# xxlong0/ESTDepth

Hardware: AMD Instinct MI355X
Metric: depth frames/sec (seq_len=5, 480x640, D=64) (higher is better)
Workload: dtype f32

## Files before the change

### estdepth_amd/csrc/conv2d_wino2.hip

```cpp
#include <hip/hip_runtime.h>
#include <stdint.h>
#include <stdlib.h>
#include <type_traits>

#include "estd_hip.h"
#include "estd_common.h"

#ifndef ESTD_C2W2ABL
#define ESTD_C2W2ABL 0
#endif

namespace {

typedef float f32x4 __attribute__((ext_vector_type(4)));
typedef float f32x2 __attribute__((ext_vector_type(2)));
typedef unsigned int u32x4 __attribute__((__vector_size__(16)));
constexpr unsigned OOB_OFFSET = 0xFFFFFF00u;

constexpr int TH = 8, TW = 16;
constexpr int TROWS = 16;
constexpr int NSTEP = 8;
#ifndef ESTD_C2W2_PFS
#define ESTD_C2W2_PFS 8
#endif
#ifndef ESTD_C2W2_WD
#define ESTD_C2W2_WD 2
#endif
#ifndef ESTD_C2W2_INLOOP
#define ESTD_C2W2_INLOOP 1
#endif
#ifndef ESTD_C2W2_INLOOP_PFS
#define ESTD_C2W2_INLOOP_PFS 4
#endif
#ifndef ESTD_C2W2_INLOOP_W0
#define ESTD_C2W2_INLOOP_W0 4
#endif
#ifndef ESTD_C2W2_SCHED
#define ESTD_C2W2_SCHED 2
#endif
constexpr int WD = ESTD_C2W2_WD, WR = 4;

__device__ __forceinline__ float4 as_float4(u32x4 v) { float4 f; __builtin_memcpy(&f, &v, 16); return f; }
__device__ __forceinline__ u32x4 as_u32x4(float4 f) { u32x4 v; __builtin_memcpy(&v, &f, 16); return v; }
__device__ __forceinline__ float4 f4_sub(float4 a, float4 b) { return make_float4(a.x - b.x, a.y - b.y, a.z - b.z, a.w - b.w); }
__device__ __forceinline__ float4 f4_add(float4 a, float4 b) { return make_float4(a.x + b.x, a.y + b.y, a.z + b.z, a.w + b.w); }
__device__ __forceinline__ __amdgpu_buffer_rsrc_t make_rsrc(const float* base, size_t elems)
{
    return __builtin_amdgcn_make_buffer_rsrc(const_cast<float*>(base), 0, (int)(elems * 4), 0x00020000);
}
__device__ __forceinline__ void lds_barrier() { asm volatile("s_waitcnt lgkmcnt(0)\n\ts_barrier" ::: "memory"); }

template <int DIL>
__global__ __launch_bounds__(256, 2) void conv2d_wino2_kernel(const estd_conv2d_desc p, int tiles_w, int tiles_h, int total_items)
{
    constexpr int IN_H = TH + 2 * DIL, IN_W = TW + 2 * DIL;
    constexpr bool INLOOP = ESTD_C2W2_INLOOP != 0 && (DIL == 1 || ESTD_C2W2_INLOOP == 2);
    constexpr int PITCH = DIL == 1 ? IN_W + 1 : IN_W;
    constexpr int SLOT_BYTES = TROWS * PITCH * 128;
    constexpr int SH_BYTES = 4 * PITCH * 128;
    constexpr int LOADERS = IN_W * 8;
    auto lds_off = [](int row, int col, int chunk) { return (row * PITCH + col) * 128 + ((chunk ^ ((col >> 1) & 7)) << 4); };
    extern __shared__ __attribute__((aligned(16))) char smem[];

    const int tid = threadIdx.x;
    const int lane = tid & 63;
    const int wave = __builtin_amdgcn_readfirstlane(tid >> 6);
    const int rpp = wave >> 1, nt = wave & 1;
    const int g = lane >> 4, i = lane & 15;
    const int blk_rp = (i >= 4 && i < 12) ? 1 : 0;
    const int cb = i < 4 ? i : i < 12 ? i - 4 : i - 8;
    const int rp = 2 * rpp + blk_rp;
    const int row_a = DIL == 1 ? 2 * rp : (rp & 1) + 4 * (rp >> 1);
    const int col_b = DIL == 1 ? 2 * cb : (cb & 1) + 4 * (cb >> 1);
    const int H = p.H, W = p.W, Cin = p.cin, Cout = p.cout;
    const int nchunks = Cin >> 5;
    const int tiles_per_group = p.N * tiles_h * tiles_w;
    const int wlane = lane * 16 + nt * 1024;

    int u, u_end;
    {
        const int G = gridDim.x, bid = blockIdx.x;
        const int r = ((G & 7) == 0) ? (bid & 7) * (G >> 3) + (bid >> 3) : bid;
        u = (int)((long long)total_items * r / G);
        u_end = (int)((long long)total_items * (r + 1) / G);
    }
    if (u >= u_end) return;

    const size_t img_in = (size_t)H * W * Cin, img_out = (size_t)H * W * Cout;
    const bool loader = tid < LOADERS;
    const int lzx = tid >> 3, lc = tid & 7;
    const int wbase = loader ? lds_off(0, lzx, lc) : 0;

    int aoff[4];
#pragma unroll
    for (int q = 0; q < 4; ++q) aoff[q] = lds_off(rp, col_b + DIL * q, g);

    auto decode = [&](int item, int& grp, int& n, int& th0, int& tw0) {
        grp = item / tiles_per_group;
        int t = item - grp * tiles_per_group;
        const int twi = t % tiles_w; t /= tiles_w;
        const int thi = t % tiles_h; n = t / tiles_h;
        th0 = thi * TH; tw0 = twi * TW;
    };
    auto brick_offsets = [&](int th0, int tw0, unsigned (&voff)[IN_H], bool enable) {
        const int gx = tw0 - DIL + lzx;
        const bool colok = enable && loader && (unsigned)gx < (unsigned)W;
        const unsigned base = (unsigned)(gx * Cin + lc * 4) * 4u;
        const unsigned rowbytes = (unsigned)(W * Cin) * 4u;
#pragma unroll
        for (int zy = 0; zy < IN_H; ++zy) {
            const int gy = th0 - DIL + zy;
            const bool rowok = (unsigned)gy < (unsigned)H;
            voff[zy] = (colok && rowok) ? base + (unsigned)gy * rowbytes : OOB_OFFSET;
        }
    };

    int grp, n, th0, tw0;
    decode(u, grp, n, th0, tw0);
    unsigned voff[IN_H];
    brick_offsets(th0, tw0, voff, true);
    __amdgpu_buffer_rsrc_t rs_in = make_rsrc(p.in + (size_t)n * img_in, img_in);
    float4 pf[IN_H];
#pragma unroll
    for (int zy = 0; zy < IN_H; ++zy) pf[zy] = as_float4(__builtin_amdgcn_raw_buffer_load_b128(rs_in, voff[zy], 0, 0));

    const size_t wgrp_elems = (size_t)nchunks * NSTEP * 4 * 2 * 256;
    float4 bq[WR][4];
    {
        const __amdgpu_buffer_rsrc_t rs_w0 = make_rsrc(p.w_wino + (size_t)grp * wgrp_elems, wgrp_elems);
#pragma unroll
        for (int s = 0; s < WD; ++s)
#pragma unroll
            for (int sw = 0; sw < 4; ++sw) bq[s][sw] = as_float4(__builtin_amdgcn_raw_buffer_load_b128(rs_w0, wlane, (s * 4 + sw) * 2048, 0));
    }
    const float floor_b = p.relu_before_residual ? 0.f : ESTD_NO_FLOOR;
    const float floor_a = p.relu_after_residual ? 0.f : ESTD_NO_FLOOR;

    int k = 0;
    if (INLOOP) {
        if (loader && !(ESTD_C2W2ABL & 2)) {
#pragma unroll
            for (int w = 0; w < 4; ++w) {
                const int a = DIL == 1 ? 2 * w : (w & 1) + 4 * (w >> 1);
                const float4 d0 = pf[a], d1 = pf[a + DIL], d2 = pf[a + 2 * DIL], d3 = pf[a + 3 * DIL];
                *reinterpret_cast<float4*>(smem + wbase + (0 * 4 + w) * PITCH * 128) = f4_sub(d0, d2);
                *reinterpret_cast<float4*>(smem + wbase + (1 * 4 + w) * PITCH * 128) = f4_add(d1, d2);
                *reinterpret_cast<float4*>(smem + wbase + (2 * 4 + w) * PITCH * 128) = f4_sub(d2, d1);
                *reinterpret_cast<float4*>(smem + wbase + (3 * 4 + w) * PITCH * 128) = f4_sub(d1, d3);
            }
        }
    }
    while (true) {
        const __amdgpu_buffer_rsrc_t rs_w = make_rsrc(p.w_wino + (size_t)grp * wgrp_elems, wgrp_elems);
        const int cbase = grp * 32 + nt * 16 + 4 * g;
        const float4 sc4 = *reinterpret_cast<const float4*>(p.scale + cbase), sh4 = *reinterpret_cast<const float4*>(p.shift + cbase);
        f32x4 acc[4][4];

        const bool has_next_item = (u + 1 < u_end);
        int ngrp = grp, nn_ = n, nth0 = th0, ntw0 = tw0;
        if (has_next_item) decode(u + 1, ngrp, nn_, nth0, ntw0);
        const __amdgpu_buffer_rsrc_t rs_wni = make_rsrc(p.w_wino + (size_t)ngrp * wgrp_elems, wgrp_elems);

        auto write_rows = [&](char* slot, int w0, int w1) {
            if (loader && !(ESTD_C2W2ABL & 2)) {
#pragma unroll
                for (int w = 0; w < 4; ++w) {
                    if (w < w0 || w >= w1) continue;
                    const int a = DIL == 1 ? 2 * w : (w & 1) + 4 * (w >> 1);
                    const float4 d0 = pf[a], d1 = pf[a + DIL], d2 = pf[a + 2 * DIL], d3 = pf[a + 3 * DIL];
                    *reinterpret_cast<float4*>(slot + wbase + (0 * 4 + w) * PITCH * 128) = f4_sub(d0, d2);
                    *reinterpret_cast<float4*>(slot + wbase + (1 * 4 + w) * PITCH * 128) = f4_add(d1, d2);
                    *reinterpret_cast<float4*>(slot + wbase + (2 * 4 + w) * PITCH * 128) = f4_sub(d2, d1);
                    *reinterpret_cast<float4*>(slot + wbase + (3 * 4 + w) * PITCH * 128) = f4_sub(d1, d3);
                }
            }
        };
        auto write_row_sh = [&](char* slot, int w, int sh_) {
            if (loader && !(ESTD_C2W2ABL & 2)) {
                const int a = DIL == 1 ? 2 * w : (w & 1) + 4 * (w >> 1);
                const float4 d0 = pf[a], d1 = pf[a + DIL], d2 = pf[a + 2 * DIL], d3 = pf[a + 3 * DIL];
                const float4 v = sh_ == 0 ? f4_sub(d0, d2) : sh_ == 1 ? f4_add(d1, d2) : sh_ == 2 ? f4_sub(d2, d1) : f4_sub(d1, d3);
                *reinterpret_cast<float4*>(slot + wbase + (sh_ * 4 + w) * PITCH * 128) = v;
            }
        };
        auto chunk_body = [&](auto first_c, const int c) {
            constexpr bool FIRST = decltype(first_c)::value;
            const int sb = (k & 1) * SLOT_BYTES;
            char* slot = smem + sb;
            if (!INLOOP) write_rows(slot, 0, 4);
            lds_barrier();

            const bool last_chunk = (c + 1 == nchunks);
            int pf_soff = (c + 1) * 128;
            if (last_chunk) {
                brick_offsets(nth0, ntw0, voff, has_next_item);
                if (nn_ != n) rs_in = make_rsrc(p.in + (size_t)nn_ * img_in, img_in);
                pf_soff = 0;
            }
            const int wbase_q = c * NSTEP * 4;
            const __amdgpu_buffer_rsrc_t rs_wx = last_chunk ? rs_wni : rs_w;
            const int wnext_q = last_chunk ? 0 : wbase_q + NSTEP * 4;

            int ao[4];
#pragma unroll
            for (int q = 0; q < 4; ++q) ao[q] = aoff[q] + sb;
            auto load_rows = [&](int st, float4 (&Rr)[4]) {
#pragma unroll
                for (int q = 0; q < 4; ++q)
                    Rr[q] = *reinterpret_cast<const float4*>(smem + ((st & 1) ? (ao[q] ^ 64) : ao[q]) + (st >> 1) * SH_BYTES);
            };
            auto xform2 = [&](const float4 (&Rr)[4], int h, f32x2 (&o)[4]) {
                f32x2 r[4];
#pragma unroll
                for (int q = 0; q < 4; ++q) r[q] = h == 0 ? (f32x2){Rr[q].x, Rr[q].y} : (f32x2){Rr[q].z, Rr[q].w};
                if (ESTD_C2W2ABL & 128) { o[0] = r[0]; o[1] = r[1]; o[2] = r[2]; o[3] = r[3]; }
                else { o[0] = r[0] - r[2]; o[1] = r[1] + r[2]; o[2] = r[2] - r[1]; o[3] = r[1] - r[3]; }
            };
            f32x2 T[2][4];
            float4 R[4];
            load_rows(0, R);
            xform2(R, 0, T[0]);
            xform2(R, 1, T[1]);
            load_rows(1, R);
            __builtin_amdgcn_sched_barrier(0);

#pragma clang loop unroll(full)
            for (int st = 0; st < NSTEP; ++st) {
                const int sh = st >> 1;
                f32x2 Tn[2][4];
                if (ESTD_C2W2_SCHED == 2) {
                    constexpr int PFS = INLOOP ? ESTD_C2W2_INLOOP_PFS : ESTD_C2W2_PFS;
                    const int r0 = PFS != 8 ? (st < PFS ? st * IN_H / PFS : IN_H) : DIL == 1 ? (st == 0 ? 0 : st + 1) : (3 * st + 1) / 2;
                    const int r1 = PFS != 8 ? (st < PFS ? (st + 1) * IN_H / PFS : IN_H)
                                            : DIL == 1 ? ((st == 0 || st == NSTEP - 1) ? r0 + 2 : r0 + 1) : (3 * (st + 1) + 1) / 2;
                    const bool wr = INLOOP && st >= ESTD_C2W2_INLOOP_W0 && (!last_chunk || has_next_item);
                    constexpr int WN = NSTEP - ESTD_C2W2_INLOOP_W0;
                    static_assert(!INLOOP || WN == 4, "quarter schedule: one row pair of the next chunk per step");
#pragma unroll
                    for (int h = 0; h < 2; ++h) {
#pragma unroll
                        for (int e = 0; e < 2; ++e) {
                            const int qk = 2 * h + e;
                            if (!(ESTD_C2W2ABL & 8)) {
                                const int tgt = st + WD;
                                bq[tgt % WR][qk] = tgt < NSTEP
                                    ? as_float4(__builtin_amdgcn_raw_buffer_load_b128(rs_w, wlane, (wbase_q + tgt * 4 + qk) * 2048, 0))
                                    : as_float4(__builtin_amdgcn_raw_buffer_load_b128(rs_wx, wlane, (wnext_q + (tgt - NSTEP) * 4 + qk) * 2048, 0));
                            }
#pragma unroll
                            for (int r = r0 + (r1 - r0) * qk / 4; r < r0 + (r1 - r0) * (qk + 1) / 4; ++r)
                                pf[r] = as_float4(__builtin_amdgcn_raw_buffer_load_b128(rs_in, voff[r], pf_soff, 0));
                            if (wr) write_row_sh(smem + (((k + 1) & 1) * SLOT_BYTES), st - ESTD_C2W2_INLOOP_W0, qk);
                            __builtin_amdgcn_sched_barrier(0);
#pragma unroll
                            for (int sw = 0; sw < 4; ++sw) {
                                const float4 b4 = bq[(ESTD_C2W2ABL & 8) ? 0 : st % WR][sw];
                                const float b = h == 0 ? (e == 0 ? b4.x : b4.y) : (e == 0 ? b4.z : b4.w);
                                const bool first_product = FIRST && (st & 1) == 0 && h == 0 && e == 0;
                                const f32x4 c_in = first_product ? (f32x4){0.f, 0.f, 0.f, 0.f} : acc[sh][sw];
                                acc[sh][sw] = __builtin_amdgcn_mfma_f32_16x16x4f32(b, T[h][sw][e], c_in, 0, 0, 0);
                            }
                            if (e == 1 && st + 1 < NSTEP) xform2(R, h, Tn[h]);
                            __builtin_amdgcn_sched_barrier(0);
                        }
                    }
                } else {
                if (!(ESTD_C2W2ABL & 8)) {
                    const int tgt = st + WD;
#pragma unroll
                    for (int sw = 0; sw < 4; ++sw)
                        bq[tgt % WR][sw] = tgt < NSTEP
                            ? as_float4(__builtin_amdgcn_raw_buffer_load_b128(rs_w, wlane, (wbase_q + tgt * 4 + sw) * 2048, 0))
                            : as_float4(__builtin_amdgcn_raw_buffer_load_b128(rs_wx, wlane, (wnext_q + (tgt - NSTEP) * 4 + sw) * 2048, 0));
                }
                {
                    constexpr int PFS = INLOOP ? ESTD_C2W2_INLOOP_PFS : ESTD_C2W2_PFS;
                    const int r0 = PFS != 8 ? (st < PFS ? st * IN_H / PFS : IN_H) : DIL == 1 ? (st == 0 ? 0 : st + 1) : (3 * st + 1) / 2;
                    const int r1 = PFS != 8 ? (st < PFS ? (st + 1) * IN_H / PFS : IN_H)
                                            : DIL == 1 ? ((st == 0 || st == NSTEP - 1) ? r0 + 2 : r0 + 1) : (3 * (st + 1) + 1) / 2;
#pragma unroll
                    for (int r = r0; r < r1; ++r) pf[r] = as_float4(__builtin_amdgcn_raw_buffer_load_b128(rs_in, voff[r], pf_soff, 0));
                }
                if (INLOOP && st >= ESTD_C2W2_INLOOP_W0 && (!last_chunk || has_next_item)) {
                    constexpr int WN = NSTEP - ESTD_C2W2_INLOOP_W0;
                    const int i0 = (st - ESTD_C2W2_INLOOP_W0) * 4 / WN, i1 = (st - ESTD_C2W2_INLOOP_W0 + 1) * 4 / WN;
                    write_rows(smem + (((k + 1) & 1) * SLOT_BYTES), i0, i1);
                }
                if (!ESTD_C2W2_SCHED) __builtin_amdgcn_sched_barrier(0);
#pragma unroll
                for (int h = 0; h < 2; ++h) {
#pragma unroll
                    for (int e = 0; e < 2; ++e)
#pragma unroll
                        for (int sw = 0; sw < 4; ++sw) {
                            const float4 b4 = bq[(ESTD_C2W2ABL & 8) ? 0 : st % WR][sw];
                            const float b = h == 0 ? (e == 0 ? b4.x : b4.y) : (e == 0 ? b4.z : b4.w);
                            const bool first_product = FIRST && (st & 1) == 0 && h == 0 && e == 0;
                            const f32x4 c_in = first_product ? (f32x4){0.f, 0.f, 0.f, 0.f} : acc[sh][sw];
                            acc[sh][sw] = __builtin_amdgcn_mfma_f32_16x16x4f32(b, T[h][sw][e], c_in, 0, 0, 0);
                        }
                    if (st + 1 < NSTEP) xform2(R, h, Tn[h]);
                }
                }
                if (st + 2 < NSTEP) load_rows(st + 2, R);
                if (ESTD_C2W2_SCHED == 2) {
                    __builtin_amdgcn_sched_group_barrier(0x100, 4, 0);
                } else if (ESTD_C2W2_SCHED) {
#pragma unroll
                    for (int i = 0; i < 8; ++i) {
                        __builtin_amdgcn_sched_group_barrier(0x008, 2, 0);
                        __builtin_amdgcn_sched_group_barrier(0x020, 1, 0);
                        __builtin_amdgcn_sched_group_barrier(0x200, 1, 0);
                        __builtin_amdgcn_sched_group_barrier(0x002, 4, 0);
                    }
                    __builtin_amdgcn_sched_group_barrier(0x100, 4, 0);
                } else {
#pragma unroll
                    for (int h = 0; h < 2; ++h) {
                        __builtin_amdgcn_sched_group_barrier(0x008, 8, 0);
                        __builtin_amdgcn_sched_group_barrier(0x002, 4, 0);
                    }
                    __builtin_amdgcn_sched_group_barrier(0x100, 4, 0);
                }
                if (st + 1 < NSTEP) {
#pragma unroll
                    for (int h = 0; h < 2; ++h)
#pragma unroll
                        for (int sw = 0; sw < 4; ++sw) T[h][sw] = Tn[h][sw];
                }
                __builtin_amdgcn_sched_barrier(0);
            }
        };
        chunk_body(std::true_type{}, 0);
        ++k;
        for (int c = 1; c < nchunks; ++c, ++k) chunk_body(std::false_type{}, c);

        auto epilogue = [&](auto has_res_c) {
            constexpr bool HAS_RES = decltype(has_res_c)::value;
            const __amdgpu_buffer_rsrc_t rs_out = make_rsrc(p.out + (size_t)n * img_out, img_out);
            const __amdgpu_buffer_rsrc_t rs_res = make_rsrc((HAS_RES ? p.residual : p.out) + (size_t)n * img_out, img_out);
            const float floor_1 = HAS_RES ? floor_b : fmaxf(floor_b, floor_a);
            unsigned eo[2][2];
#pragma unroll
            for (int r = 0; r < 2; ++r)
#pragma unroll
                for (int j = 0; j < 2; ++j) {
                    const int y = th0 + row_a + DIL * r, x = tw0 + col_b + DIL * j;
                    eo[r][j] = (y < H && x < W) ? (unsigned)((y * W + x) * Cout + cbase) * 4u : OOB_OFFSET;
                }
            float4 res[2][2];
            if (HAS_RES) {
#pragma unroll
                for (int r = 0; r < 2; ++r)
#pragma unroll
                    for (int j = 0; j < 2; ++j) res[r][j] = as_float4(__builtin_amdgcn_raw_buffer_load_b128(rs_res, eo[r][j], 0, 0));
            }
            f32x4 z[4][2];
#pragma unroll
            for (int s = 0; s < 4; ++s) {
                z[s][0] = acc[s][0] + acc[s][1] + acc[s][2];
                z[s][1] = acc[s][1] - acc[s][2] - acc[s][3];
            }
#pragma unroll
            for (int r = 0; r < 2; ++r)
#pragma unroll
                for (int j = 0; j < 2; ++j) {
                    const f32x4 yv = r == 0 ? z[0][j] + z[1][j] + z[2][j] : z[1][j] - z[2][j] - z[3][j];
                    float4 v;
                    v.x = fmaxf(fmaf(yv[0], sc4.x, sh4.x), floor_1); v.y = fmaxf(fmaf(yv[1], sc4.y, sh4.y), floor_1);
                    v.z = fmaxf(fmaf(yv[2], sc4.z, sh4.z), floor_1); v.w = fmaxf(fmaf(yv[3], sc4.w, sh4.w), floor_1);
                    if (HAS_RES) {
                        v.x = fmaxf(v.x + res[r][j].x, floor_a); v.y = fmaxf(v.y + res[r][j].y, floor_a);
                        v.z = fmaxf(v.z + res[r][j].z, floor_a); v.w = fmaxf(v.w + res[r][j].w, floor_a);
                    }
                    if (ESTD_C2W2ABL & 1) asm volatile("" :: "v"(v.x), "v"(v.w));
                    else __builtin_amdgcn_raw_buffer_store_b128(as_u32x4(v), rs_out, eo[r][j], 0, 0);
                }
        };
        if (p.residual) epilogue(std::true_type{}); else epilogue(std::false_type{});

        if (!has_next_item) break;
        ++u;
        grp = ngrp; n = nn_; th0 = nth0; tw0 = ntw0;
    }
}

}

extern "C" int estd_conv2d_k3_wino2(const estd_conv2d_desc* dp, estd_stream_t s)
{
    if (!dp) return ESTD_ERR_ARG;
    const estd_conv2d_desc& d = *dp;
    if (d.N <= 0 || d.H <= 0 || d.W <= 0 || !d.in || !d.w_wino || !d.scale || !d.shift || !d.out) return ESTD_ERR_ARG;
    if (d.cin < 32 || (d.cin & 31) || d.cout < 32 || (d.cout & 31)) return ESTD_ERR_ARG;
    if (d.dilation != 1 && d.dilation != 2) return ESTD_ERR_UNSUPPORTED;
    const long long widest = (long long)d.H * d.W * (d.cin > d.cout ? d.cin : d.cout) * 4;
    if (widest >= 0x7fffff00LL) return ESTD_ERR_UNSUPPORTED;
    const int tiles_w = (d.W + TW - 1) / TW, tiles_h = (d.H + TH - 1) / TH;
    const int groups = d.cout / 32;
    const long long total = (long long)groups * d.N * tiles_h * tiles_w;
    if (total > 0x7fffffffLL) return ESTD_ERR_ARG;
    const int slots = estd_persistent_wgs(2);
    int grid = total < slots ? (int)total : slots;
    if (grid >= 8) grid &= ~7;
    if (d.dilation == 1) {
        const size_t lds = (size_t)2 * TROWS * (TW + 3) * 128;
        estd_allow_dynamic_lds<conv2d_wino2_kernel<1>>((int)lds);
        hipLaunchKernelGGL(conv2d_wino2_kernel<1>, dim3(grid), dim3(256), lds, estd_stream(s), d, tiles_w, tiles_h, (int)total);
    } else {
        const size_t lds = (size_t)2 * TROWS * (TW + 4) * 128;
        estd_allow_dynamic_lds<conv2d_wino2_kernel<2>>((int)lds);
        hipLaunchKernelGGL(conv2d_wino2_kernel<2>, dim3(grid), dim3(256), lds, estd_stream(s), d, tiles_w, tiles_h, (int)total);
    }
    return ESTD_LAUNCH_CHECK();
}
```

Measured before the change: 195.8.

## Add split-wave Winograd path covering 64 output channels with half-height tiles

Adds a new kernel body that applies when cout is a multiple of 64. Each workgroup covers 64 output channels over a half-height spatial tile, so wave pairs pick different 32-channel weight groups and share the same input brick. The two row-halves of the output transform are split across waves and combined through an LDS exchange buffer. The goal is to reuse each loaded input tile across more output channels and cut per-tile LDS footprint, at the cost of an extra barrier and exchange per item and a more complex schedule.

```diff
diff --git a/estdepth_amd/csrc/conv2d_wino2.hip b/estdepth_amd/csrc/conv2d_wino2.hip
--- a/estdepth_amd/csrc/conv2d_wino2.hip
+++ b/estdepth_amd/csrc/conv2d_wino2.hip
@@ -37,6 +37,9 @@
 #endif
 #ifndef ESTD_C2W2_SCHED
 #define ESTD_C2W2_SCHED 2
+#endif
+#ifndef ESTD_C2W2_SPLIT
+#define ESTD_C2W2_SPLIT 1
 #endif
 constexpr int WD = ESTD_C2W2_WD, WR = 4;
 
@@ -51,7 +54,7 @@
 __device__ __forceinline__ void lds_barrier() { asm volatile("s_waitcnt lgkmcnt(0)\n\ts_barrier" ::: "memory"); }
 
 template <int DIL>
-__global__ __launch_bounds__(256, 2) void conv2d_wino2_kernel(const estd_conv2d_desc p, int tiles_w, int tiles_h, int total_items)
+__device__ __forceinline__ void wino2_rpp_nt(const estd_conv2d_desc& p, int tiles_w, int tiles_h, int total_items)
 {
     constexpr int IN_H = TH + 2 * DIL, IN_W = TW + 2 * DIL;
     constexpr bool INLOOP = ESTD_C2W2_INLOOP != 0 && (DIL == 1 || ESTD_C2W2_INLOOP == 2);
@@ -385,6 +388,299 @@
     }
 }
 
+template <int DIL, bool WIDE>
+__device__ __forceinline__ void wino2_split(const estd_conv2d_desc& p, int tiles_w, int tiles_h, int total_items)
+{
+    constexpr int TH_ = WIDE ? TH / 2 : TH;
+    constexpr int NP = TH_ / 2;
+    constexpr int IN_H = TH_ + 2 * DIL, IN_W = TW + 2 * DIL;
+    constexpr bool INLOOP = ESTD_C2W2_INLOOP != 0 && (DIL == 1 || ESTD_C2W2_INLOOP == 2);
+    constexpr int PITCH = DIL == 1 ? IN_W + 1 : IN_W;
+    constexpr int ROW_BYTES = PITCH * 128;
+    constexpr int SLOT_BYTES = 4 * NP * ROW_BYTES;
+    constexpr int SH_BYTES = NP * ROW_BYTES;
+    constexpr int LOADERS = IN_W * 8;
+    constexpr int NQ = 4;
+    auto lds_off = [](int row, int col, int chunk) { return row * ROW_BYTES + col * 128 + ((chunk ^ ((col >> 1) & 7)) << 4); };
+    extern __shared__ __attribute__((aligned(16))) char smem[];
+
+    const int tid = threadIdx.x;
+    const int lane = tid & 63;
+    const int wave = __builtin_amdgcn_readfirstlane(tid >> 6);
+    const int shp = wave & 1, sel = wave >> 1;
+    const int g = lane >> 4, i = lane & 15;
+    const int blk_rp = (i >= 4 && i < 12) ? 1 : 0;
+    const int cb = i < 4 ? i : i < 12 ? i - 4 : i - 8;
+    const int rp = (WIDE ? 0 : 2 * sel) + blk_rp;
+    const int row_a = DIL == 1 ? 2 * rp : (rp & 1) + 4 * (rp >> 1);
+    const int col_b = DIL == 1 ? 2 * cb : (cb & 1) + 4 * (cb >> 1);
+    const int H = p.H, W = p.W, Cin = p.cin, Cout = p.cout;
+    const int nchunks = Cin >> 5;
+    const int tiles_per_group = p.N * tiles_h * tiles_w;
+    const int wlane = lane * 16;
+    const int srec = shp * 16;
+
+    int u, u_end;
+    {
+        const int G = gridDim.x, bid = blockIdx.x;
+        const int r = ((G & 7) == 0) ? (bid & 7) * (G >> 3) + (bid >> 3) : bid;
+        u = (int)((long long)total_items * r / G);
+        u_end = (int)((long long)total_items * (r + 1) / G);
+    }
+    if (u >= u_end) return;
+
+    const size_t img_in = (size_t)H * W * Cin, img_out = (size_t)H * W * Cout;
+    const bool loader = tid < LOADERS;
+    const int lzx = tid >> 3, lc = tid & 7;
+    const int wbase = loader ? lds_off(0, lzx, lc) : 0;
+
+    int aoff[4];
+#pragma unroll
+    for (int q = 0; q < 4; ++q) aoff[q] = lds_off(rp, col_b + DIL * q, g);
+
+    auto decode = [&](int item, int& grp, int& n, int& th0, int& tw0) {
+        grp = item / tiles_per_group;
+        int t = item - grp * tiles_per_group;
+        const int twi = t % tiles_w; t /= tiles_w;
+        const int thi = t % tiles_h; n = t / tiles_h;
+        th0 = thi * TH_; tw0 = twi * TW;
+    };
+    auto brick_offsets = [&](int th0, int tw0, unsigned (&voff)[IN_H], bool enable) {
+        const int gx = tw0 - DIL + lzx;
+        const bool colok = enable && loader && (unsigned)gx < (unsigned)W;
+        const unsigned base = (unsigned)(gx * Cin + lc * 4) * 4u;
+        const unsigned rowbytes = (unsigned)(W * Cin) * 4u;
+#pragma unroll
+        for (int zy = 0; zy < IN_H; ++zy) {
+            const int gy = th0 - DIL + zy;
+            const bool rowok = (unsigned)gy < (unsigned)H;
+            voff[zy] = (colok && rowok) ? base + (unsigned)gy * rowbytes : OOB_OFFSET;
+        }
+    };
+
+    int grp, n, th0, tw0;
+    decode(u, grp, n, th0, tw0);
+    unsigned voff[IN_H];
+    brick_offsets(th0, tw0, voff, true);
+    __amdgpu_buffer_rsrc_t rs_in = make_rsrc(p.in + (size_t)n * img_in, img_in);
+    float4 pf[IN_H];
+#pragma unroll
+    for (int zy = 0; zy < IN_H; ++zy) pf[zy] = as_float4(__builtin_amdgcn_raw_buffer_load_b128(rs_in, voff[zy], 0, 0));
+
+    const size_t wgrp_elems = (size_t)nchunks * NSTEP * 4 * 2 * 256;
+    auto wgrp_rsrc = [&](int grp_) { return make_rsrc(p.w_wino + (size_t)(WIDE ? 2 * grp_ + sel : grp_) * wgrp_elems, wgrp_elems); };
+    float4 bw[2][4][2];
+    {
+        const __amdgpu_buffer_rsrc_t rs_w0 = wgrp_rsrc(grp);
+#pragma unroll
+        for (int sw = 0; sw < 4; ++sw)
+#pragma unroll
+            for (int t = 0; t < 2; ++t) bw[0][sw][t] = as_float4(__builtin_amdgcn_raw_buffer_load_b128(rs_w0, wlane, (srec + sw) * 2048 + t * 1024, 0));
+    }
+    const float floor_b = p.relu_before_residual ? 0.f : ESTD_NO_FLOOR;
+    const float floor_a = p.relu_after_residual ? 0.f : ESTD_NO_FLOOR;
+
+    auto write_row_sh = [&](char* slot, int w, int sh_) {
+        if (loader && !(ESTD_C2W2ABL & 2)) {
+            const int a = DIL == 1 ? 2 * w : (w & 1) + 4 * (w >> 1);
+            const float4 d0 = pf[a], d1 = pf[a + DIL], d2 = pf[a + 2 * DIL], d3 = pf[a + 3 * DIL];
+            const float4 v = sh_ == 0 ? f4_sub(d0, d2) : sh_ == 1 ? f4_add(d1, d2) : sh_ == 2 ? f4_sub(d2, d1) : f4_sub(d1, d3);
+            *reinterpret_cast<float4*>(slot + wbase + (sh_ * NP + w) * ROW_BYTES) = v;
+        }
+    };
+    auto write_rows = [&](char* slot) {
+#pragma unroll
+        for (int w = 0; w < NP; ++w)
+#pragma unroll
+            for (int s = 0; s < 4; ++s) write_row_sh(slot, w, s);
+    };
+
+    int k = 0;
+    if (INLOOP) write_rows(smem);
+    while (true) {
+        const __amdgpu_buffer_rsrc_t rs_w = wgrp_rsrc(grp);
+        const int cbase = (WIDE ? 64 * grp + 32 * sel : 32 * grp) + 4 * g;
+        f32x4 acc[2][4][2];
+
+        const bool has_next_item = (u + 1 < u_end);
+        int ngrp = grp, nn_ = n, nth0 = th0, ntw0 = tw0;
+        if (has_next_item) decode(u + 1, ngrp, nn_, nth0, ntw0);
+        const __amdgpu_buffer_rsrc_t rs_wni = wgrp_rsrc(ngrp);
+
+        auto chunk_body = [&](auto first_c, const int c) {
+            constexpr bool FIRST = decltype(first_c)::value;
+            const int sb = (k & 1) * SLOT_BYTES;
+            char* slot = smem + sb;
+            if (!INLOOP) write_rows(slot);
+            lds_barrier();
+
+            const bool last_chunk = (c + 1 == nchunks);
+            int pf_soff = (c + 1) * 128;
+            if (last_chunk) {
+                brick_offsets(nth0, ntw0, voff, has_next_item);
+                if (nn_ != n) rs_in = make_rsrc(p.in + (size_t)nn_ * img_in, img_in);
+                pf_soff = 0;
+            }
+            const int wrec = c * NSTEP * 4 + srec;
+            const __amdgpu_buffer_rsrc_t rs_wx = last_chunk ? rs_wni : rs_w;
+            const int wrec_x = (last_chunk ? 0 : (c + 1) * NSTEP * 4) + srec;
+
+            int ao[4];
+#pragma unroll
+            for (int q = 0; q < 4; ++q) ao[q] = aoff[q] + sb + 2 * shp * SH_BYTES;
+            auto load_rows = [&](int L, float4 (&Rr)[4]) {
+#pragma unroll
+                for (int q = 0; q < 4; ++q)
+                    Rr[q] = *reinterpret_cast<const float4*>(smem + ((L & 1) ? (ao[q] ^ 64) : ao[q]) + (L >> 1) * SH_BYTES);
+            };
+            auto xform2 = [&](const float4 (&Rr)[4], int h, f32x2 (&o)[4]) {
+                f32x2 r[4];
+#pragma unroll
+                for (int q = 0; q < 4; ++q) r[q] = h == 0 ? (f32x2){Rr[q].x, Rr[q].y} : (f32x2){Rr[q].z, Rr[q].w};
+                if (ESTD_C2W2ABL & 128) { o[0] = r[0]; o[1] = r[1]; o[2] = r[2]; o[3] = r[3]; }
+                else { o[0] = r[0] - r[2]; o[1] = r[1] + r[2]; o[2] = r[2] - r[1]; o[3] = r[1] - r[3]; }
+            };
+            f32x2 T[2][4];
+            float4 R[4];
+            load_rows(0, R);
+            xform2(R, 0, T[0]);
+            xform2(R, 1, T[1]);
+            load_rows(1, R);
+            __builtin_amdgcn_sched_barrier(0);
+
+#pragma clang loop unroll(full)
+            for (int L = 0; L < NQ; ++L) {
+                const int sl = L >> 1;
+                f32x2 Tn[2][4];
+#pragma unroll
+                for (int q = 0; q < 4; ++q) {
+                    const int j = NQ * L + q;
+                    if (!(ESTD_C2W2ABL & 8)) {
+#pragma unroll
+                        for (int t = 0; t < 2; ++t)
+                            bw[(L + 1) & 1][q][t] = L + 1 < NQ
+                                ? as_float4(__builtin_amdgcn_raw_buffer_load_b128(rs_w, wlane, (wrec + (L + 1) * 4 + q) * 2048 + t * 1024, 0))
+                                : as_float4(__builtin_amdgcn_raw_buffer_load_b128(rs_wx, wlane, (wrec_x + q) * 2048 + t * 1024, 0));
+                    }
+                    constexpr int NJ = INLOOP ? 2 * 4 : NQ * 4;
+#pragma unroll
+                    for (int r = IN_H * j / NJ; r < (j < NJ ? IN_H * (j + 1) / NJ : 0); ++r)
+                        pf[r] = as_float4(__builtin_amdgcn_raw_buffer_load_b128(rs_in, voff[r], pf_soff, 0));
+                    if (INLOOP && L >= 2 && (!last_chunk || has_next_item)) {
+                        char* nslot = smem + ((k + 1) & 1) * SLOT_BYTES;
+                        const int jw = j - 8;
+                        if (WIDE) write_row_sh(nslot, jw >> 2, jw & 3);
+                        else { write_row_sh(nslot, jw >> 1, 2 * (jw & 1)); write_row_sh(nslot, jw >> 1, 2 * (jw & 1) + 1); }
+                    }
+                    __builtin_amdgcn_sched_barrier(0);
+#pragma unroll
+                    for (int h = 0; h < 2; ++h)
+#pragma unroll
+                        for (int e = 0; e < 2; ++e)
+#pragma unroll
+                            for (int t = 0; t < 2; ++t) {
+                                const float4 b4 = bw[(ESTD_C2W2ABL & 8) ? 0 : L & 1][q][t];
+                                const float b = h == 0 ? (e == 0 ? b4.x : b4.y) : (e == 0 ? b4.z : b4.w);
+                                const bool first_product = FIRST && (L & 1) == 0 && h == 0 && e == 0;
+                                const f32x4 c_in = first_product ? (f32x4){0.f, 0.f, 0.f, 0.f} : acc[sl][q][t];
+                                acc[sl][q][t] = __builtin_amdgcn_mfma_f32_16x16x4f32(b, T[h][q][e], c_in, 0, 0, 0);
+                            }
+                    if ((q & 1) && L + 1 < NQ) xform2(R, q >> 1, Tn[q >> 1]);
+                    __builtin_amdgcn_sched_barrier(0);
+                }
+                if (L + 2 < NQ) load_rows(L + 2, R);
+                __builtin_amdgcn_sched_group_barrier(0x100, 4, 0);
+                if (L + 1 < NQ) {
+#pragma unroll
+                    for (int h = 0; h < 2; ++h)
+#pragma unroll
+                        for (int sw = 0; sw < 4; ++sw) T[h][sw] = Tn[h][sw];
+                }
+                __builtin_amdgcn_sched_barrier(0);
+            }
+        };
+        chunk_body(std::true_type{}, 0);
+        ++k;
+        for (int c = 1; c < nchunks; ++c, ++k) chunk_body(std::false_type{}, c);
+
+        const float4 sc4[2] = {*reinterpret_cast<const float4*>(p.scale + cbase), *reinterpret_cast<const float4*>(p.scale + cbase + 16)};
+        const float4 sh4[2] = {*reinterpret_cast<const float4*>(p.shift + cbase), *reinterpret_cast<const float4*>(p.shift + cbase + 16)};
+        f32x4 z[2][2][2];
+#pragma unroll
+        for (int sl = 0; sl < 2; ++sl)
+#pragma unroll
+            for (int t = 0; t < 2; ++t) {
+                z[sl][0][t] = acc[sl][0][t] + acc[sl][1][t] + acc[sl][2][t];
+                z[sl][1][t] = acc[sl][1][t] - acc[sl][2][t] - acc[sl][3][t];
+            }
+        char* xb = WIDE ? smem + 2 * SLOT_BYTES : smem + ((k - 1) & 1) * SLOT_BYTES;
+        if (!WIDE) lds_barrier();
+#pragma unroll
+        for (int v = 0; v < 4; ++v)
+            *reinterpret_cast<f32x4*>(xb + wave * 4096 + (v * 64 + lane) * 16) = shp == 0 ? z[1][v >> 1][v & 1] : z[0][v >> 1][v & 1];
+        lds_barrier();
+        f32x4 zo[2][2];
+#pragma unroll
+        for (int v = 0; v < 4; ++v) zo[v >> 1][v & 1] = *reinterpret_cast<const f32x4*>(xb + (wave ^ 1) * 4096 + (v * 64 + lane) * 16);
+
+        auto epilogue = [&](auto has_res_c) {
+            constexpr bool HAS_RES = decltype(has_res_c)::value;
+            const __amdgpu_buffer_rsrc_t rs_out = make_rsrc(p.out + (size_t)n * img_out, img_out);
+            const __amdgpu_buffer_rsrc_t rs_res = make_rsrc((HAS_RES ? p.residual : p.out) + (size_t)n * img_out, img_out);
+            const float floor_1 = HAS_RES ? floor_b : fmaxf(floor_b, floor_a);
+            const int y = th0 + row_a + DIL * shp;
+            unsigned eo[2][2];
+#pragma unroll
+            for (int j = 0; j < 2; ++j)
+#pragma unroll
+                for (int t = 0; t < 2; ++t) {
+                    const int x = tw0 + col_b + DIL * j;
+                    eo[j][t] = (y < H && x < W) ? (unsigned)((y * W + x) * Cout + cbase + 16 * t) * 4u : OOB_OFFSET;
+                }
+            float4 res[2][2];
+            if (HAS_RES) {
+#pragma unroll
+                for (int j = 0; j < 2; ++j)
+#pragma unroll
+                    for (int t = 0; t < 2; ++t) res[j][t] = as_float4(__builtin_amdgcn_raw_buffer_load_b128(rs_res, eo[j][t], 0, 0));
+            }
+#pragma unroll
+            for (int j = 0; j < 2; ++j)
+#pragma unroll
+                for (int t = 0; t < 2; ++t) {
+                    const f32x4 yv = shp == 0 ? z[0][j][t] + z[1][j][t] + zo[j][t] : zo[j][t] - z[0][j][t] - z[1][j][t];
+                    float4 v;
+                    v.x = fmaxf(fmaf(yv[0], sc4[t].x, sh4[t].x), floor_1); v.y = fmaxf(fmaf(yv[1], sc4[t].y, sh4[t].y), floor_1);
+                    v.z = fmaxf(fmaf(yv[2], sc4[t].z, sh4[t].z), floor_1); v.w = fmaxf(fmaf(yv[3], sc4[t].w, sh4[t].w), floor_1);
+                    if (HAS_RES) {
+                        v.x = fmaxf(v.x + res[j][t].x, floor_a); v.y = fmaxf(v.y + res[j][t].y, floor_a);
+                        v.z = fmaxf(v.z + res[j][t].z, floor_a); v.w = fmaxf(v.w + res[j][t].w, floor_a);
+                    }
+                    if (ESTD_C2W2ABL & 1) asm volatile("" :: "v"(v.x), "v"(v.w));
+                    else __builtin_amdgcn_raw_buffer_store_b128(as_u32x4(v), rs_out, eo[j][t], 0, 0);
+                }
+        };
+        if (p.residual) epilogue(std::true_type{}); else epilogue(std::false_type{});
+
+        if (!has_next_item) break;
+        ++u;
+        grp = ngrp; n = nn_; th0 = nth0; tw0 = ntw0;
+    }
+}
+
+template <int DIL>
+__global__ __launch_bounds__(256, 2) void conv2d_wino2_kernel(const estd_conv2d_desc p, int tiles_w, int tiles_h, int total_items)
+{
+#if ESTD_C2W2_SPLIT
+    if ((p.cout & 63) == 0) { wino2_split<DIL, true>(p, tiles_w, tiles_h, total_items); return; }
+#endif
+#if ESTD_C2W2_SPLIT == 2
+    wino2_split<DIL, false>(p, tiles_w, tiles_h, total_items);
+#else
+    wino2_rpp_nt<DIL>(p, tiles_w, tiles_h, total_items);
+#endif
+}
+
 }
 
 extern "C" int estd_conv2d_k3_wino2(const estd_conv2d_desc* dp, estd_stream_t s)
@@ -396,20 +692,23 @@
     if (d.dilation != 1 && d.dilation != 2) return ESTD_ERR_UNSUPPORTED;
     const long long widest = (long long)d.H * d.W * (d.cin > d.cout ? d.cin : d.cout) * 4;
     if (widest >= 0x7fffff00LL) return ESTD_ERR_UNSUPPORTED;
-    const int tiles_w = (d.W + TW - 1) / TW, tiles_h = (d.H + TH - 1) / TH;
-    const int groups = d.cout / 32;
+    const bool wide = ESTD_C2W2_SPLIT != 0 && (d.cout & 63) == 0;
+    const int th = wide ? TH / 2 : TH;
+    const int tiles_w = (d.W + TW - 1) / TW, tiles_h = (d.H + th - 1) / th;
+    const int groups = d.cout / (wide ? 64 : 32);
     const long long total = (long long)groups * d.N * tiles_h * tiles_w;
     if (total > 0x7fffffffLL) return ESTD_ERR_ARG;
     const int slots = estd_persistent_wgs(2);
     int grid = total < slots ? (int)total : slots;
     if (grid >= 8) grid &= ~7;
+    const size_t rows = wide ? TROWS / 2 : TROWS, xchg = wide ? 16384 : 0;
     if (d.dilation == 1) {
-        const size_t lds = (size_t)2 * TROWS * (TW + 3) * 128;
-        estd_allow_dynamic_lds<conv2d_wino2_kernel<1>>((int)lds);
+        const size_t lds = 2 * rows * (TW + 3) * 128 + xchg;
+        estd_allow_dynamic_lds<conv2d_wino2_kernel<1>>(2 * TROWS * (TW + 3) * 128);
         hipLaunchKernelGGL(conv2d_wino2_kernel<1>, dim3(grid), dim3(256), lds, estd_stream(s), d, tiles_w, tiles_h, (int)total);
     } else {
-        const size_t lds = (size_t)2 * TROWS * (TW + 4) * 128;
-        estd_allow_dynamic_lds<conv2d_wino2_kernel<2>>((int)lds);
+        const size_t lds = 2 * rows * (TW + 4) * 128 + xchg;
+        estd_allow_dynamic_lds<conv2d_wino2_kernel<2>>(2 * TROWS * (TW + 4) * 128);
         hipLaunchKernelGGL(conv2d_wino2_kernel<2>, dim3(grid), dim3(256), lds, estd_stream(s), d, tiles_w, tiles_h, (int)total);
     }
     return ESTD_LAUNCH_CHECK();
```

New measurement: 200.0 (median of 6 runs). +2.1%, better.
